# dmlc/difacto

Hardware: AMD Instinct MI355X
Metric: examples/sec (FM SGD worker step, Criteo-shape, V_dim=64) (higher is better)
Workload: dtype f32

## Files before the change

difacto_amd/capi.py:

```python
import ctypes as C
import os

import numpy as np

_HERE = os.path.dirname(os.path.abspath(__file__))
LIB_PATH = os.environ.get("DIFACTO_HIP_LIB") or os.path.join(_HERE, "libdifacto_hip.so")

FEA_COUNT, WEIGHT, GRADIENT = 1, 2, 3
INIT_REFRAND, INIT_HASH = 0, 1
U64MAX = 2 ** 64 - 1

SYMBOLS = [
    "dfh_last_error", "dfh_updater_param_default", "dfh_ctx_create", "dfh_ctx_destroy", "dfh_ctx_sync",
    "dfh_ctx_stream", "dfh_ctx_device", "dfh_reverse_bytes", "dfh_encode_fea_grp_id", "dfh_table_create",
    "dfh_table_destroy", "dfh_table_size", "dfh_table_param", "dfh_table_bytes", "dfh_pull", "dfh_push",
    "dfh_table_export", "dfh_table_import", "dfh_fm_predict", "dfh_fm_calcgrad", "dfh_loss_evaluate",
    "dfh_auc_times_n", "dfh_batch_create", "dfh_batch_destroy", "dfh_batch_load_host", "dfh_batch_load_device",
    "dfh_localize", "dfh_batch_load_localized_host", "dfh_batch_get_localized", "dfh_batch_shape", "dfh_sgd_step",
    "dfh_batch_progress", "dfh_batch_get_pred", "dfh_row_stride", "dfh_shard_pull", "dfh_shard_push_count",
    "dfh_shard_push_grad", "dfh_batch_forward", "dfh_batch_backward", "dfh_batch_device_keys", "dfh_malloc",
    "dfh_free", "dfh_memcpy_h2d", "dfh_memcpy_d2h", "dfh_ctx_set_timing", "dfh_ctx_get_timing", "dfh_kernel_name",
    "dfh_table_warm_start", "dfh_ctx_set_pipeline", "dfh_batch_lookup", "dfh_localize_lookup", "dfh_rowbuf_create", "dfh_rowbuf_destroy", "dfh_rowbuf_load_host", "dfh_batch_gather_rows", "dfh_batch_set_option", "dfh_batch_key_ranges", "dfh_batch_attach_device",
    "dfh_batch_key_ranges_device", "dfh_shard_resolve", "dfh_shard_pull_resolved", "dfh_shard_push_count_resolved",
    "dfh_shard_push_grad_resolved", "dfh_table_check", "dfh_ctx_set_timing_mask", "dfh_table_save", "dfh_table_load", "dfh_shard_resolve_multi", "dfh_shard_push_count_multi",
    "dfh_shard_push_grad_multi", "dfh_shard_count_pull_multi", "dfh_shard_push_grad_listed", "dfh_shard_release", "dfh_ctx_set_option", "dfh_table_set_has_aux", "dfh_table_has_aux",
    "dfh_comm_unique_id", "dfh_comm_create_rccl", "dfh_comm_create_callback", "dfh_comm_destroy", "dfh_comm_rank", "dfh_comm_world",
    "dfh_comm_allreduce_sum", "dfh_shard_create", "dfh_shard_destroy", "dfh_shard_owned_range", "dfh_shard_step", "dfh_shard_prefetch_counts",
    "dfh_shard_pull_host", "dfh_shard_push_host", "dfh_comm_allgather", "dfh_shard_balanced_splits", "dfh_shard_set_exchange", "dfh_shard_set_timing", "dfh_shard_get_timing",
    "dfh_comm_stats", "dfh_comm_info", "dfh_comm_selfcheck", "dfh_comm_wire_probe", "dfh_table_capacity", "dfh_batch_prepare_rows", "dfh_rowbuf_load_host_slices",
    "dfh_rowbuf_set_labels", "dfh_batch_prepare_cached", "dfh_batch_get_rows",
    "dfh_batch_create_many", "dfh_shard_multi_words", "dfh_shard_reserve", "dfh_comm_create_loopback", "dfh_comm_loopback_feed", "dfh_comm_loopback_wire", "dfh_comm_loopback_wire_time",
    "dfh_vec_inner_multi", "dfh_vec_combine", "dfh_vec_line_step", "dfh_lbfgs_create", "dfh_lbfgs_destroy", "dfh_lbfgs_add_chunk",
    "dfh_lbfgs_init_model", "dfh_lbfgs_shape", "dfh_lbfgs_get_model", "dfh_lbfgs_set_weights", "dfh_lbfgs_calc_grad",
    "dfh_lbfgs_prepare_direction", "dfh_lbfgs_calc_direction", "dfh_lbfgs_line_search", "dfh_lbfgs_evaluate", "dfh_lbfgs_create_sharded",
    "dfh_lbfgs_owned_range", "dfh_lbfgs_set_model", "dfh_bcd_set_model",
    "dfh_bcd_create", "dfh_bcd_destroy", "dfh_bcd_add_chunk", "dfh_bcd_build", "dfh_bcd_shape", "dfh_bcd_block_info",
    "dfh_bcd_epoch", "dfh_bcd_step", "dfh_bcd_get_model", "dfh_bcd_get_pred", "dfh_batch_split_entries",
    "dfh_bcd_create_sharded",
    "dfh_textchunk_create", "dfh_textchunk_destroy", "dfh_textchunk_parse_criteo", "dfh_textchunk_rows", "dfh_textchunk_ids",
    "dfh_rowbuf_load_slices",
]
XCHG_COUNTS, XCHG_KEYS, XCHG_CNT, XCHG_ROWS, XCHG_GRADS, XCHG_OTHER = range(6)
SHARD_STAGES = ("counts", "L", "K", "R", "RW", "F", "G", "P")
K_COUNT = 8
K_LOCALIZE, K_LOOKUP, K_FORWARD, K_BACKWARD, K_PULL, K_PUSH, K_MISC, K_AUC = range(8)


class UpdaterParam(C.Structure):
    _fields_ = [("l1", C.c_float), ("l2", C.c_float), ("V_l2", C.c_float), ("lr", C.c_float),
                ("lr_beta", C.c_float), ("V_lr", C.c_float), ("V_lr_beta", C.c_float),
                ("V_init_scale", C.c_float), ("V_dim", C.c_int), ("V_threshold", C.c_int),
                ("seed", C.c_uint), ("init_mode", C.c_int)]
# ... 56 lines not shown
    L.dfh_table_capacity.argtypes = [vp, PP(u64), PP(u64)]
    L.dfh_table_bytes.restype = u64
    L.dfh_table_bytes.argtypes = [vp]
    L.dfh_pull.argtypes = [vp, vp, sz, vp, PP(sz), vp, PP(sz)]
    L.dfh_push.argtypes = [vp, vp, sz, i32, vp, sz, vp, sz]
    L.dfh_table_export.argtypes = [vp, u64, vp, vp, vp, vp, PP(u64)]
    L.dfh_table_import.argtypes = [vp, u64, vp, vp, vp, vp]
    L.dfh_fm_predict.argtypes = [vp, i32, sz, vp, vp, vp, vp, sz, vp, vp, sz, vp]
    L.dfh_fm_calcgrad.argtypes = [vp, i32, sz, vp, vp, vp, vp, vp, sz, vp, vp, sz, vp, vp]
    L.dfh_loss_evaluate.argtypes = [vp, vp, vp, sz, PP(f32)]
    L.dfh_auc_times_n.argtypes = [vp, vp, vp, sz, PP(f32)]
    L.dfh_batch_create.argtypes = [vp, sz, sz, PP(vp)]
    L.dfh_batch_destroy.argtypes = [vp]
    L.dfh_batch_create_many.argtypes = [vp, i32, sz, sz, PP(vp)]
    L.dfh_batch_split_entries.argtypes = [vp, vp]
    L.dfh_batch_load_host.argtypes = [vp, sz, vp, vp, vp, vp]
    L.dfh_batch_load_device.argtypes = [vp, sz, sz, vp, vp, vp, vp]
    L.dfh_batch_attach_device.argtypes = [vp, sz, sz, vp, vp, vp, vp]
    L.dfh_localize.argtypes = [vp, u64]
    L.dfh_batch_load_localized_host.argtypes = [vp, sz, vp, vp, vp, vp, vp, vp, sz]
    L.dfh_batch_get_localized.argtypes = [vp, PP(sz), vp, vp, vp]
    L.dfh_batch_shape.argtypes = [vp, PP(sz), PP(sz), PP(sz)]
    L.dfh_sgd_step.argtypes = [vp, vp, i32, i32]
    L.dfh_batch_progress.argtypes = [vp, PP(Progress), i32]
    L.dfh_batch_get_pred.argtypes = [vp, vp]
    L.dfh_row_stride.restype = sz
    L.dfh_row_stride.argtypes = [i32]
    L.dfh_shard_pull.argtypes = [vp, vp, sz, vp]
    L.dfh_shard_push_count.argtypes = [vp, vp, sz, vp]
    L.dfh_shard_push_grad.argtypes = [vp, vp, sz, vp]
# ... 554 lines not shown
        p = Progress()
        _ck(lib().dfh_batch_progress(self.h, C.byref(p), 1 if reset else 0))
        return p

    def pred(self):
        nrows, _, _ = self.shape(want_U=False)
        out = np.zeros(nrows, np.float32)
        _ck(lib().dfh_batch_get_pred(self.h, _p(out)))
        return out

    def split_entries(self):
        n = C.c_uint32(0)
        _ck(lib().dfh_batch_split_entries(self.h, C.byref(n)))
        return int(n.value)

    def forward(self, V_dim, d_rows):
        _ck(lib().dfh_batch_forward(self.h, V_dim, _dp(d_rows)))

    def backward(self, V_dim, d_rows, d_grads):
        _ck(lib().dfh_batch_backward(self.h, V_dim, _dp(d_rows), _dp(d_grads)))

    def key_ranges(self, nparts):
        out = np.zeros(nparts + 1, np.uint32)
        _ck(lib().dfh_batch_key_ranges(self.h, nparts, _p(out)))
        return out

    def device_keys(self):
        a, b, u = C.c_void_p(), C.c_void_p(), C.c_size_t(0)
        _ck(lib().dfh_batch_device_keys(self.h, C.byref(a), C.byref(b), C.byref(u)))
        return a.value, b.value, u.value
# ... 388 lines not shown
```

difacto_amd/csrc/dfh_api.hip:

```cpp
#include <algorithm>
#include <chrono>
#include <cstring>
#include <mutex>
#include <new>
#include <thread>

#include <hip/hip_ext.h>
#include <rocprim/rocprim.hpp>

#include "dfh_kernels.hip"
#include "dfh_localize.hip"
#include "dfh_update.hip"
#include "dfh_riders.hip"

using namespace dfh;

namespace dfh {
static thread_local std::string g_err;
void set_error(const std::string& msg) { g_err = msg; }
}

struct dfh_ctx {
  int device = 0;
  hipStream_t stream = nullptr;
  bool own_stream = false;
  std::vector<hipStream_t> preps;
  std::vector<hipStream_t> extra;
  hipStream_t parse = nullptr;
  std::mutex parse_mu;
  unsigned nprep = 0;
  unsigned next_prep = 0;
  bool pipeline = false;
  void* scratch = nullptr;
  size_t scratch_bytes = 0;
  int num_cu = 256;
  int fwd_depth = 5;
  int fwd_blocks = 0;
  int bwd_small_blocks = 2048;
  int upd_kernel = 1;
  int upd_hot_blocks = 512, upd_mid_blocks = 512, upd_few_blocks = 1024, upd_single_blocks = 4096;
  int upd_interleave = 0;
  int owner_per_key = 0;
  int upd_split = 1;
  int auc_in_update = 1;
  int shard_mixed_update = 1;
  int grow_initial_rows = 1 << 20;
  int event_flags = 1;
  int prep_priority = -1;
  int single_queue = 0;
  int rider_slot[4] = {2, 0, 1, 2};
  int rider_alone[4] = {0, 0, 0, 0};
  int rider_period[3] = {1, 1, 1};
// ... 104 lines not shown
  uint32_t* d_split_ticket = nullptr;
  float* d_split_part = nullptr;
  size_t split_cap = 0;
  int split_sel = 0, split_last = 0;
  bool split_listing = false;
  uint32_t seg_nb = 0;
  uint2* d_uw = nullptr;
  uint32_t *d_urow = nullptr, *d_need = nullptr, *d_rank = nullptr, *d_total = nullptr;
  float *d_pred = nullptr, *d_slope = nullptr, *d_xv = nullptr;
  size_t xv_floats = 0;
  static constexpr size_t kProgDoubles = 2 * PROG_SLOTS + 64;
  double* d_prog = nullptr;
  float nrows_seen = 0;
  hipEvent_t ev_ready = nullptr, ev_free = nullptr;
  bool ready_pending = false, free_pending = false;
  hipStream_t prep = nullptr;
  bool compute_auc = false;
  uint32_t *d_auc_keys = nullptr, *d_auc_skeys = nullptr, *d_auc_lab = nullptr, *d_auc_slab = nullptr;
  uint32_t* d_auc_part = nullptr;
  uint32_t auc_pending_n = 0;
  bool force_radix = false;
  bool force_sort_fallback = false;
  dfh_table* looked_up = nullptr;
  struct GatherSeg { struct dfh_rowbuf* rb; size_t at, n; };
  std::vector<GatherSeg> gsegs;
  GatherSrc gsrc{};
  bool gather_pending = false, gather_fusable = false, gather_any_value = false, loc_fuse_gather = false;
  const uint32_t *g_rows = nullptr, *g_off = nullptr;
  const float* g_lab = nullptr;
  LocView loc_v{};
  EmitOut loc_o{};
// ... 3 lines not shown
};

namespace dfh {
namespace chunks {
inline hipError_t reset_prog(dfh_batch* b, hipStream_t s);
}
}

namespace {
int flush_pending(dfh_batch* b);
void pend_remove(dfh_ctx* c, dfh_batch* b);
inline hipStream_t prep_of(const dfh_batch* b) {
  const dfh_ctx* c = b->ctx;
  return (c->pipeline && b->prep) ? b->prep : c->stream;
}
void phase_begin(dfh_batch* b) {
  dfh_ctx* c = b->ctx;
  if (b->pend_stage < RID_STAGES) (void)flush_pending(b);
  hipStream_t next = c->pipeline ? c->preps[c->next_prep++ % c->nprep] : nullptr;
  if (next && b->prep && next != b->prep && b->ready_pending) {
    (void)hipStreamWaitEvent(next, b->ev_ready, 0);
  }
  b->prep = next;
}
int prep_begin(dfh_batch* b) {
  dfh_ctx* c = b->ctx;
  if (c->pipeline && !b->prep) phase_begin(b);
  if (c->pipeline && b->free_pending) {
    DFH_HIP(hipStreamWaitEvent(prep_of(b), b->ev_free, 0));
    b->free_pending = false;
  }
  return DFH_OK;
}
int prep_end(dfh_batch* b) {
  dfh_ctx* c = b->ctx;
  if (c->pipeline && !b->defer_ready) {
    DFH_HIP(hipEventRecord(b->ev_ready, prep_of(b)));
    b->ready_pending = true;
  }
  return DFH_OK;
}
int main_begin(dfh_batch* b) {
  dfh_ctx* c = b->ctx;
  if (b->pend_stage < RID_STAGES) {
    int rc = flush_pending(b);
    if (rc) return rc;
  }
  if (b->ready_pending) {
    DFH_HIP(hipStreamWaitEvent(c->stream, b->ev_ready, 0));
    b->ready_pending = false;
  }
  return DFH_OK;
}
int main_end(dfh_batch* b) {
  dfh_ctx* c = b->ctx;
  if (b->split_listing) {
    b->split_listing = false;
    b->split_last = b->split_sel;
    b->split_sel ^= 1;
  }
  if (c->pipeline) {
    DFH_HIP(hipEventRecord(b->ev_free, c->stream));
    b->free_pending = true;
// ... 14 lines not shown
  return SplitOut{b->d_split_ent, split_counter(b), u_base, (uint32_t)b->split_cap};
}
}

namespace {

inline int grid_for_threads(size_t n, const dfh_ctx* c) {
  size_t b = (n + 255) / 256;
  size_t cap = (size_t)c->num_cu * 8;
  return (int)std::max<size_t>(1, std::min(b, cap));
}
inline int grid_for_waves(size_t nwaves, const dfh_ctx* c) {
  size_t b = (nwaves + 3) / 4;
  size_t cap = (size_t)c->num_cu * 8;
  return (int)std::max<size_t>(1, std::min(b, cap));
}

int ensure_scratch(dfh_ctx* c, size_t bytes) {
  if (bytes <= c->scratch_bytes) return DFH_OK;
  if (c->scratch) {
    DFH_HIP(hipStreamSynchronize(c->stream));
    DFH_HIP(hipFree(c->scratch));
    c->scratch = nullptr;
    c->scratch_bytes = 0;
  }
  size_t want = std::max(bytes, (size_t)1 << 20);
  want = (want + 255) & ~(size_t)255;
  DFH_HIP(hipMalloc(&c->scratch, want));
  c->scratch_bytes = want;
  return DFH_OK;
// ... 486 lines not shown

inline int count_mode(const dfh_ctx* c, int is_train, int push_cnt) { return push_cnt ? ((is_train && c->upd_kernel) ? 2 : 1) : 0; }

struct StepExtras {
  uint32_t* need = nullptr;
  bool pre = false;
  bool riders = false;
  bool spans = false;
};

int step_lookup(dfh_table* t, dfh_batch* b, int is_train, int push_cnt, uint32_t lo, const uint32_t* d_n, size_t n, const StepExtras& x,
                const float* rrows = nullptr, size_t U = 0, hipEvent_t rows_in = nullptr) {
  dfh_ctx* c = t->ctx;
  hipStream_t s = c->stream;
  const float* cnt = b->has_cnt ? b->d_feacnt + lo : (const float*)nullptr;
  const int mode = count_mode(c, is_train, push_cnt), gl = grid_for_threads(n, c);
  const uint32_t n_static = d_n ? 0u : (uint32_t)n;
  static const bool gap_trace = getenv("DFH_GAP_TRACE") != nullptr;
  const bool ride = x.spans && gap_trace && ((c->timing >> DFH_K_LOOKUP) & 1u);
  TimeScope ts(c, (x.spans && !ride) ? DFH_K_LOOKUP : DFH_K_COUNT);
  const SplitOut so = split_out(c, b, is_train, lo);
  RiderSet rs;
  rs.n = 0;
  if (x.riders) collect_riders(c, 0, true, ((uint32_t)gl + 7u) / 8u, &rs);
  if (rrows) {
    DFH_HIP(hipStreamWaitEvent(s, rows_in, 0));
    const UwRemote m{rrows, dfh_row_stride(t->v.k), b->d_U, lo, lo + (uint32_t)n, b->d_uw, b->d_col_ptr, split_out(c, b, is_train, 0u), t->v.err};
    hipLaunchKernelGGL(k_lookup_uw_remote, dim3(grid_for_threads(U, c)), dim3(256), 0, s, t->v, b->d_feaids + lo, n_static, b->d_urow + lo,
                       cnt, b->d_col_ptr + lo, mode, b->d_uw + lo, auc_pending(b), m, so);
  } else if (rs.n) {
    hipLaunchKernelGGL(k_lookup_riders, dim3((((unsigned)gl + 7u) / 8u + rs.ngroups) * 8u), dim3(256), rider_smem(rs), s, t->v,
// ... 156 lines not shown
  delete c;
  return DFH_OK;
}

int dfh_ctx_sync(dfh_ctx* c) {
  DFH_ARG(c, "ctx is NULL");
  return sync_all(c);
}

int dfh_ctx_set_pipeline(dfh_ctx* c, int enable) {
  DFH_ARG(c, "ctx is NULL");
  DFH_ARG(enable >= 0 && enable <= 4, "dfh_ctx_set_pipeline: 0 (off) .. 4 preparation streams");
  if (c->single_queue && enable) {
    return DFH_OK;
  }
  int rc = sync_all(c);
  if (rc) return rc;
  while ((int)c->preps.size() < enable) {
    int lo = 0, hi = 0;
    DFH_HIP(hipDeviceGetStreamPriorityRange(&lo, &hi));
    const int prio = c->prep_priority < 0 ? lo : (c->prep_priority > 0 ? hi : 0);
    hipStream_t p = nullptr;
    DFH_HIP(hipStreamCreateWithPriority(&p, hipStreamNonBlocking, prio));
    c->preps.push_back(p);
  }
  c->nprep = (unsigned)enable;
  c->next_prep = 0;
  c->pipeline = enable != 0;
  return DFH_OK;
}
int dfh_ctx_set_option(dfh_ctx* c, const char* name, int value) {
  DFH_ARG(c && name, "dfh_ctx_set_option: NULL argument");
  const std::string n(name);
  if (n == "fwd_depth") {
    DFH_ARG(value == 4 || value == 5 || value == 8 || value == 10, "fwd_depth must be 4, 5, 8 or 10");
    c->fwd_depth = value;
  } else if (n == "fwd_blocks") {
    DFH_ARG(value >= 0 && value <= PROG_SLOTS, "fwd_blocks must be in [0, 16384] (0: one wave per example)");
    c->fwd_blocks = value;
  } else if (n == "bwd_small_blocks") {
    DFH_ARG(value >= 1 && value <= 65536, "bwd_small_blocks must be in [1, 65536]");
    c->bwd_small_blocks = value;
  } else if (n == "upd_kernel") {
    DFH_ARG(value == 0 || value == 1, "upd_kernel must be 0 (k_backward_all) or 1 (k_update_fused)");
    c->upd_kernel = value;
  } else if (n == "upd_hot_blocks" || n == "upd_mid_blocks" || n == "upd_few_blocks" || n == "upd_single_blocks") {
    DFH_ARG(value >= 1 && value <= 65536, "upd_*_blocks must be in [1, 65536]");
    (n == "upd_hot_blocks" ? c->upd_hot_blocks : n == "upd_mid_blocks" ? c->upd_mid_blocks : n == "upd_few_blocks" ? c->upd_few_blocks
                                                                                                        : c->upd_single_blocks) = value;
  } else if (n == "grow_initial_rows") {
    DFH_ARG(value >= 16 && value <= (1 << 28), "grow_initial_rows must be in [16, 2^28]");
    c->grow_initial_rows = value;
  } else if (n == "auc_in_update") {
    DFH_ARG(value == 0 || value == 1, "auc_in_update must be 0 (k_auc_pairs as its own launch) or 1 (a role of k_update_fused)");
// ... 8 lines not shown
    DFH_ARG(value == 0 || value == 1, "upd_split must be 0 (one block per hot key, whatever its length) or 1 (a block per part of 1 024 occurrences)");
    c->upd_split = value;
  } else if (n == "upd_interleave") {
    DFH_ARG(value >= 0 && value <= 64, "upd_interleave must be in [0, 64]");
    c->upd_interleave = value;
  } else if (n == "event_flags") {
    DFH_ARG(value == 0 || value == 1, "event_flags must be 0 (default events) or 1 (no system-scope fence); set before batches are created");
    c->event_flags = value;
  } else if (n == "single_queue") {
    DFH_ARG(value == 0 || value == 1, "single_queue must be 0 (preparation streams) or 1 (the Localizer's stages ride in the step's launches)");
    if (value != c->single_queue) {
      for (dfh_batch* p : std::vector<dfh_batch*>(c->pend)) {
        int rcf = flush_pending(p);
        if (rcf) return rcf;
      }
      int rcs = sync_all(c);
      if (rcs) return rcs;
      if (value) {
        c->nprep = 0;
        c->next_prep = 0;
        c->pipeline = false;
      }
      c->single_queue = value;
    }
  } else if (n == "rider_slot_count" || n == "rider_slot_scatter" || n == "rider_slot_sort" || n == "rider_slot_emit") {
    DFH_ARG(value >= 0 && value <= 6 && (value & 3) <= 2, "rider_slot_*: 0 lookup, 1 forward, 2 update (+ 4: alone, before that launch)");
    const int st = n == "rider_slot_count" ? 0 : n == "rider_slot_scatter" ? 1 : n == "rider_slot_sort" ? 2 : 3;
    c->rider_slot[st] = value & 3;
    c->rider_alone[st] = (value >> 2) & 1;
  } else if (n == "rider_start_lookup" || n == "rider_start_forward" || n == "rider_start_update") {
    DFH_ARG(value >= 0 && value <= 100, "rider_start_*: per cent of the carrier's own blocks dispatched before the first rider group");
// ... 1124 lines not shown
  }
  if (--sa->refs == 0) {
    hipFree(sa->base);
    delete sa;
  }
  return rc;
}

int dfh_batch_destroy(dfh_batch* b) {
  if (b && b->n_prof)
    fprintf(stderr, "dfh_batch_prepare_rows x %llu: begin %.4f s, wait staged %.4f, write description %.4f, gather %.4f, localize %.4f, lookup + ready %.4f\n",
            (unsigned long long)b->n_prof, b->t_prof[0], b->t_prof[1], b->t_prof[2], b->t_prof[3], b->t_prof[4], b->t_prof[5]);
  if (!b) return DFH_OK;
  hipSetDevice(b->ctx->device);
  pend_remove(b->ctx, b);
  sync_all(b->ctx);
  if (b->ev_ready) hipEventDestroy(b->ev_ready);
  if (b->ev_free) hipEventDestroy(b->ev_free);
  if (b->ev_staged) hipEventDestroy(b->ev_staged);
  if (b->h_stage) hipHostFree(b->h_stage);
  if (b->d_xv) hipFree(b->d_xv);
  if (b->arena) hipFree(b->arena);
  if (b->shared_arena) {
    SharedArena* sa = static_cast<SharedArena*>(b->shared_arena);
    if (--sa->refs == 0) {
      hipFree(sa->base);
      delete sa;
    }
  }
  delete b;
// ... 292 lines not shown
  } else {
    hipLaunchKernelGGL(k_rdx_keys, dim3(g), dim3(256), 0, s, b->d_raw, N, max_index, b->d_keys, b->d_pos);
    size_t tb = b->temp_bytes;
    DFH_HIP(rocprim::radix_sort_pairs(b->d_temp, tb, b->d_keys, b->d_skeys, b->d_pos, b->d_spos, (size_t)N, 0, 64, s));
    hipLaunchKernelGGL(k_rdx_heads, dim3(g), dim3(256), 0, s, b->d_skeys, N, b->d_head);
    tb = b->temp_bytes;
    DFH_HIP(rocprim::inclusive_scan(b->d_temp, tb, b->d_head, b->d_uid, (size_t)N, rocprim::plus<uint32_t>(), s));
    hipLaunchKernelGGL(k_rdx_emit, dim3(g), dim3(256), 0, s, b->d_skeys, b->d_spos, b->d_head, b->d_uid, N, (uint32_t)b->nrows,
                       b->d_offset, b->has_value ? b->d_value : (const float*)nullptr, b->d_feaids, b->d_col_ptr, b->d_index,
                       b->d_s_row, b->d_s_val, b->d_U);
    hipLaunchKernelGGL(k_seg_lists_reset, dim3(1), dim3(64), 0, s, b->d_mid, b->d_hot, b->d_few, b->d_U + 2);
    hipLaunchKernelGGL(k_seg_lists, dim3((unsigned)std::max<size_t>(1, std::min<size_t>((N + 1023) / 1024, 256))), dim3(1024), 0, s,
                       b->d_col_ptr, b->d_U, b->d_mid, b->d_hot, b->d_few, b->d_mid_ent, b->d_hot_ent, b->d_few_ent);
    b->seg_nb = 1;
    if (probe)
      hipLaunchKernelGGL(k_lookup, dim3(grid_for_threads(b->nnz, c)), dim3(256), 0, s, probe->v, b->d_feaids, b->d_U, 0u, b->d_urow,
                         (const float*)nullptr, b->d_col_ptr, 0, (uint32_t*)nullptr, 0, (uint2*)nullptr, AucFin{nullptr, 0u, nullptr});
  }
  delete tsp;
  DFH_HIP(hipGetLastError());
  b->localized = true;
  b->has_cnt = false;
  if (probe) b->looked_up = probe;
  return prep_end(b);
}
}


int dfh_localize(dfh_batch* b, uint64_t max_index) {
  DFH_ARG(b && b->nrows > 0, "dfh_localize: no batch loaded");
  DFH_ARG(max_index != 0, "max_index must be nonzero");
// ... 35 lines not shown
    set_error("dfh_batch_lookup: batch is not localized");
    return DFH_ERR_STATE;
  }
  dfh_ctx* c = b->ctx;
  if (b->nnz == 0) return DFH_OK;
  if (b->nnz <= kSmallBatchPairs) return DFH_OK;
  if (c->single_queue) return DFH_OK;
  DFH_HIP(hipSetDevice(c->device));
  int rc = table_reserve(t, b->nnz);
  if (rc) return rc;
  rc = prep_begin(b);
  if (rc) return rc;
  {
    hipStream_t ps = prep_of(b);
    TimeScope ts(c, DFH_K_LOOKUP, ps);
    hipLaunchKernelGGL(k_lookup, dim3(grid_for_threads(b->nnz, c)), dim3(256), 0, ps, t->v, b->d_feaids, b->d_U, 0u,
                       b->d_urow, (const float*)nullptr, b->d_col_ptr, 0, (uint32_t*)nullptr, 0, (uint2*)nullptr, AucFin{nullptr, 0u, nullptr});
  }
  DFH_HIP(hipGetLastError());
  b->looked_up = t;
  return prep_end(b);
}

int dfh_batch_load_localized_host(dfh_batch* b, size_t nrows, const size_t* offset, const uint32_t* index, const float* value,
                                  const float* label, const uint64_t* feaids, const float* feacnt, size_t U) {
  DFH_ARG(b && offset && label && feaids, "dfh_batch_load_localized_host: NULL argument");
  DFH_ARG(nrows >= 1 && nrows <= b->max_rows, "nrows out of range");
  std::vector<uint32_t> off32;
  int rc = to_u32_offsets(offset, nrows, &off32);
  if (rc) return rc;
  const size_t base = offset[0], nnz = off32[nrows];
// ... 37 lines not shown
  DFH_HIP(hipMemcpyAsync(b->d_label, label, nrows * 4, hipMemcpyHostToDevice, s));
  if (U) DFH_HIP(hipMemcpyAsync(b->d_feaids, feaids, U * 8, hipMemcpyHostToDevice, s));
  if (U && feacnt) DFH_HIP(hipMemcpyAsync(b->d_feacnt, feacnt, U * 4, hipMemcpyHostToDevice, s));
  DFH_HIP(hipMemcpyAsync(b->d_col_ptr, col_ptr.data(), (U + 1) * 4, hipMemcpyHostToDevice, s));
  DFH_HIP(hipMemcpyAsync(b->d_U, &U32, 4, hipMemcpyHostToDevice, s));
  hipLaunchKernelGGL(k_seg_lists_reset, dim3(1), dim3(64), 0, s, b->d_mid, b->d_hot, b->d_few, b->d_U + 2);
  if (U) {
    hipLaunchKernelGGL(k_seg_lists, dim3((unsigned)std::min<size_t>((U + 1023) / 1024, 256)), dim3(1024), 0, s, b->d_col_ptr,
                       b->d_U, b->d_mid, b->d_hot, b->d_few, b->d_mid_ent, b->d_hot_ent, b->d_few_ent);
  }
  b->seg_nb = 1;
  DFH_HIP(hipGetLastError());
  DFH_HIP(hipStreamSynchronize(s));
  b->nrows = nrows;
  b->nnz = nnz;
  b->has_value = value != nullptr;
  b->has_cnt = feacnt != nullptr;
  b->localized = true;
  return prep_end(b);
}

int dfh_batch_shape(dfh_batch* b, size_t* nrows, size_t* nnz, size_t* U) {
  DFH_ARG(b, "NULL batch");
  if (nrows) *nrows = b->nrows;
  if (nnz) *nnz = b->nnz;
  if (U) {
    DFH_ARG(b->localized, "batch is not localized");
    uint32_t u = 0;
    int rc = flush_pending(b);
    if (rc) return rc;
    rc = sync_all(b->ctx);
    if (rc) return rc;
    DFH_HIP(hipMemcpyAsync(&u, b->d_U, 4, hipMemcpyDeviceToHost, b->ctx->stream));
    DFH_HIP(hipStreamSynchronize(b->ctx->stream));
    *U = u;
  }
  return DFH_OK;
}

int dfh_batch_get_localized(dfh_batch* b, size_t* U, uint64_t* feaids, float* feacnt, uint32_t* index) {
  DFH_ARG(b && b->localized, "batch is not localized");
  size_t u = 0;
  int rc = dfh_batch_shape(b, nullptr, nullptr, &u);
  if (rc) return rc;
  if (U) *U = u;
  hipStream_t s = b->ctx->stream;
  if (feaids && u) DFH_HIP(hipMemcpyAsync(feaids, b->d_feaids, u * 8, hipMemcpyDeviceToHost, s));
  if (feacnt && u) {
    if (!b->has_cnt) {
      hipLaunchKernelGGL(k_loc_counts, dim3(grid_for_threads(u, b->ctx)), dim3(256), 0, s, b->d_col_ptr, b->d_U, b->d_feacnt);
// ... 109 lines not shown
  if (is_train && refrand) {
    rc = refrand_flush(t, b->d_feaids, b->d_U, Nb, b->d_urow, b->d_need, b->d_rank, b->d_total);
    if (rc) return rc;
  }
  return main_end(b);
}

int dfh_batch_split_entries(dfh_batch* b, uint32_t* n) {
  DFH_ARG(b && n, "dfh_batch_split_entries: NULL argument");
  dfh_ctx* c = b->ctx;
  DFH_HIP(hipSetDevice(c->device));
  if (b->pend_stage < RID_STAGES) {
    int rc = flush_pending(b);
    if (rc) return rc;
  }
  if (b->ready_pending) DFH_HIP(hipStreamWaitEvent(c->stream, b->ev_ready, 0));
  DFH_HIP(hipMemcpyAsync(n, b->d_U + 2 + b->split_last, sizeof(uint32_t), hipMemcpyDeviceToHost, c->stream));
  DFH_HIP(hipStreamSynchronize(c->stream));
  return DFH_OK;
}

int dfh_batch_forward(dfh_batch* b, int V_dim, const float* d_rows) {
  DFH_ARG(b && b->localized && d_rows, "dfh_batch_forward: bad argument");
  const int kp = (V_dim + 3) / 4 * 4;
  int rc = ensure_xv(b, kp);
  if (rc) return rc;
  b->nrows_seen += (float)b->nrows;
  rc = main_begin(b);
  if (rc) return rc;
  rc = launch_forward(b, packed_src(d_rows, V_dim), V_dim, kp);
  if (rc) return rc;
  return main_end(b);
// ... 100 lines not shown
```

difacto_amd/csrc/dfh_feed.hip:

```cpp
struct dfh_rowbuf {
  dfh_ctx* ctx = nullptr;
  size_t max_rows = 0, max_nnz = 0, nrows = 0, nnz = 0;
  uint32_t* d_off = nullptr;
  uint64_t* d_idx = nullptr;
  float* d_val = nullptr;
  float* d_lab = nullptr;
  bool has_value = false, has_labels = false;
  hipStream_t up = nullptr;
  hipEvent_t ev_loaded = nullptr;
  struct Used { hipStream_t stream; hipEvent_t ev; bool pending; };
  std::mutex mu;
  std::vector<Used> used;
  std::vector<hipStream_t> seen_loaded;
  double t_prof[3] = {0, 0, 0};
  uint64_t n_prof = 0, bytes_prof = 0;
  std::vector<uint32_t> off32;
};

namespace {
int localize_impl(dfh_batch* b, uint64_t max_index, dfh_table* probe);

struct PrepLaps {
  double* acc;
  bool on;
// ... 303 lines not shown
  gs.dst_off = b->d_offset;
  gs.dst_lab = b->d_label;
  batch_loaded(b, nrows, in.nnz, in.any_value);
  return DFH_OK;
}

int queue_described(dfh_table* t, dfh_batch* b, const DescribedIn& in, uint64_t max_index, PrepLaps& laps) {
  dfh_ctx* c = b->ctx;
  int rc = describe(b, in);
  if (rc) return rc;
  laps.lap(3);
  b->defer_ready = true;
  rc = localize_impl(b, max_index, nullptr);
  laps.lap(4);
  if (!rc && in.nnz > kSmallBatchPairs && !c->single_queue) {
    hipLaunchKernelGGL(k_lookup, dim3(grid_for_threads(b->nnz, c)), dim3(256), 0, prep_of(b), t->v, b->d_feaids, b->d_U, 0u, b->d_urow,
                       (const float*)nullptr, b->d_col_ptr, 0, (uint32_t*)nullptr, 0, (uint2*)nullptr, AucFin{nullptr, 0u, nullptr});
    if (hipGetLastError() != hipSuccess) rc = DFH_ERR_HIP;
    b->looked_up = t;
  }
  b->defer_ready = false;
  if (rc) return rc;
  rc = prep_end(b);
  laps.lap(5);
  if (laps.on) ++b->n_prof;
  return rc;
}
}

extern "C" {

// ... 224 lines not shown
```

difacto_amd/csrc/dfh_internal.h:

```cpp
#ifndef DFH_INTERNAL_H_
#define DFH_INTERNAL_H_
#include <hip/hip_runtime.h>
#include <stdint.h>
#include <string>
#include <vector>

#include "difacto_hip.h"

namespace dfh {

constexpr int kWave = 64;
constexpr uint64_t kEmptyKey = ~0ULL;
constexpr uint32_t kNoRow = ~0u;

struct __attribute__((aligned(16))) HEntry {
  uint64_t key;
  uint32_t row;
  uint32_t pad;
};

struct __attribute__((aligned(32))) RowHdr {
  float w;
  uint32_t has_V;
  float sqrt_g;
// ... 28 lines not shown
  const uint2* few;
  const SegEnt* few_ent;
  const SegEnt* split_ent;
  const uint32_t* split_n;
};
#ifndef DFH_HOT_SPLIT
#define DFH_HOT_SPLIT 1024
#endif
#ifndef DFH_HOT_SPLIT_MIN
#define DFH_HOT_SPLIT_MIN 4096
#endif
constexpr uint32_t HOT_SPLIT = DFH_HOT_SPLIT;
constexpr uint32_t HOT_SPLIT_MIN = DFH_HOT_SPLIT_MIN;
#ifndef DFH_HOT_SPLIT_BUILD
#define DFH_HOT_SPLIT_BUILD 3
#endif

constexpr uint32_t kRemoteRow = 0x80000000u;
constexpr uint32_t kSingleRow = 0x40000000u;
constexpr uint32_t kCountLater = 0x20000000u;
constexpr uint32_t kHasV = 0x10000000u;
constexpr uint32_t kRowMask = 0x0FFFFFFFu;

struct RowSrc {
  const float* wbase;
  size_t wstride;
  const float* vbase;
  size_t vstride;
  const uint32_t* urow;
  int flag_is_float;
// ... 59 lines not shown
```

difacto_amd/csrc/dfh_kernels.hip:

```cpp
#include "dfh_internal.h"

namespace dfh {

__device__ __forceinline__ int lane_id() { return threadIdx.x & 63; }

__device__ __forceinline__ float wave_sum(float v) {
#pragma unroll
  for (int o = 32; o > 0; o >>= 1) v += __shfl_xor(v, o, 64);
  return v;
}

template <int L>
__device__ __forceinline__ float cross_group_sum(float v) {
#pragma unroll
  for (int o = L; o < 64; o <<= 1) v += __shfl_xor(v, o, 64);
  return v;
}
template <int L>
__device__ __forceinline__ float in_group_sum(float v) {
#pragma unroll
  for (int o = L >> 1; o > 0; o >>= 1) v += __shfl_xor(v, o, 64);
  return v;
}

// ... 379 lines not shown
  uint32_t cap;
};
__device__ __forceinline__ uint32_t* split_other(uint32_t* n) { return reinterpret_cast<uint32_t*>(reinterpret_cast<uintptr_t>(n) ^ 4u); }
__device__ __forceinline__ void lookup_split(const SplitOut& so, uint32_t* err, uint32_t u, uint32_t beg, uint32_t end) {
  if (!(DFH_HOT_SPLIT_BUILD & 1) || !so.ent || end - beg <= HOT_SPLIT_MIN) return;
  const uint32_t nparts = (end - beg + HOT_SPLIT - 1u) / HOT_SPLIT;
  const uint32_t base = atomicAdd(so.n, nparts);
  if (base + nparts > so.cap) {
    atomicOr(err, 16u);
    return;
  }
  for (uint32_t p = 0; p < nparts; ++p)
    so.ent[base + p] = make_uint4(u + so.u_base, beg + p * HOT_SPLIT, min(beg + (p + 1u) * HOT_SPLIT, end), (p << 16) | nparts);
}

template <bool SPLIT = true>
__device__ __forceinline__ void lookup_body(const TableView& t, const uint64_t* __restrict__ keys, const uint32_t* __restrict__ d_n,
                         uint32_t n_static, uint32_t* __restrict__ urow, const float* __restrict__ cnt,
                         const uint32_t* __restrict__ col_ptr, int push_cnt, uint32_t* __restrict__ need_init,
                         int rows_known, uint2* __restrict__ uw, AucFin fin, const uint32_t bid, const uint32_t nblk,
                         const SplitOut so = SplitOut{nullptr, nullptr, 0u, 0u}) {
  if (fin.n && bid == 0) auc_finalize_block(fin);
  if (SPLIT && so.n && bid == 0 && threadIdx.x == 0) *split_other(so.n) = 0u;
  uint32_t n = d_n ? *d_n : n_static;
  __shared__ uint32_t ins_sh[8];
  for (uint32_t u0 = bid * blockDim.x; u0 < n; u0 += nblk * blockDim.x) {
    const uint32_t u = u0 + threadIdx.x;
    const bool active = u < n;
    uint64_t key = active ? keys[u] : 0ull;
    uint32_t r;
    if (rows_known) r = active ? (urow[u] & kRowMask) : 0u;
    else if (blockDim.x == 256) r = find_or_insert_block(t, key, active, ins_sh);
    else r = active ? find_or_insert(t, key) : 0u;
    if (!active) continue;
    if (urow && !rows_known) urow[u] = r;
    if (SPLIT && col_ptr) lookup_split(so, t.err, u, col_ptr[u], col_ptr[u + 1]);
    float w = 0.f;
    bool hasv = false;
    if (push_cnt) {
// ... 29 lines not shown
      uw[u] = make_uint2(r | (single ? kSingleRow : 0u) | (hasv ? kHasV : 0u), __float_as_uint(w));
    }
  }
}

__global__ void k_lookup(TableView t, const uint64_t* __restrict__ keys, const uint32_t* __restrict__ d_n,
                         uint32_t n_static, uint32_t* __restrict__ urow, const float* __restrict__ cnt,
                         const uint32_t* __restrict__ col_ptr, int push_cnt, uint32_t* __restrict__ need_init,
                         int rows_known, uint2* __restrict__ uw, AucFin fin) {
  lookup_body<false>(t, keys, d_n, n_static, urow, cnt, col_ptr, push_cnt, need_init, rows_known, uw, fin, blockIdx.x, gridDim.x);
}
__global__ void k_lookup_step(TableView t, const uint64_t* __restrict__ keys, const uint32_t* __restrict__ d_n,
                              uint32_t n_static, uint32_t* __restrict__ urow, const float* __restrict__ cnt,
                              const uint32_t* __restrict__ col_ptr, int push_cnt, uint32_t* __restrict__ need_init,
                              int rows_known, uint2* __restrict__ uw, AucFin fin, SplitOut so) {
  lookup_body<true>(t, keys, d_n, n_static, urow, cnt, col_ptr, push_cnt, need_init, rows_known, uw, fin, blockIdx.x, gridDim.x, so);
}

struct UwRemote {
  const float* rows;
  size_t stride;
  const uint32_t* d_U;
  uint32_t lo, hi;
  uint2* uw;
  const uint32_t* col_ptr;
  SplitOut so;
  uint32_t* err;
};
__device__ __forceinline__ void uw_remote_body(const UwRemote& m) {
  const uint32_t U = *m.d_U;
  if (m.so.n && blockIdx.x == 0 && threadIdx.x == 0) *split_other(m.so.n) = 0u;
// ... 1711 lines not shown
```

difacto_amd/csrc/dfh_shard.hip:

```cpp
#ifndef DFH_SHARD_HIP_
#define DFH_SHARD_HIP_
#include <dlfcn.h>
#include <link.h>

#include <chrono>
#include <deque>
#include <optional>
#include <thread>

namespace dfh {

struct RcclId { char internal[128]; };
struct RcclApi {
  void* lib = nullptr;
  int (*GetUniqueId)(RcclId*) = nullptr;
  int (*CommInitRank)(void**, int, RcclId, int) = nullptr;
  int (*CommDestroy)(void*) = nullptr;
  const char* (*GetErrorString)(int) = nullptr;
  int (*Send)(const void*, size_t, int, int, void*, hipStream_t) = nullptr;
  int (*Recv)(void*, size_t, int, int, void*, hipStream_t) = nullptr;
  int (*GroupStart)() = nullptr;
  int (*GroupEnd)() = nullptr;
  int (*GetVersion)(int*) = nullptr;
  std::string path;
// ... 1066 lines not shown
int shard_step_overlap(dfh_shard* s, dfh_batch* b, int is_train, int push_cnt, int* any_active) {
  dfh_comm* c = s->c;
  dfh_ctx* ctx = s->t->ctx;
  DFH_HIP(hipSetDevice(ctx->device));
  hipStream_t st = ctx->stream, cs = s->cs;
  int rc;
  if (s->timing) ++s->stage_steps;
  static const bool trace = getenv("DFH_SHARD_TRACE") != nullptr;
  Flight& cur = s->fl[s->cur];
  if (trace)
    fprintf(stderr, "[shard %d] step %llu: b=%p cur{slot %d described %d pulled %d b=%p} armed %d next_b=%p\n", c->rank,
            (unsigned long long)s->steps, (void*)b, s->cur, (int)cur.described, (int)cur.pulled, (void*)cur.b, (int)s->next_armed,
            (void*)s->next_b);
  if (!(cur.described && cur.b == b)) {
    DFH_ARG(!cur.described || !cur.pulled, "dfh_shard_step: the batch differs from the one announced to dfh_shard_prefetch_counts");
    if (b && b->ready_pending) DFH_HIP(hipStreamWaitEvent(cs, b->ev_ready, 0));
    {
      StageScope ts(s, DFH_SHARD_STAGE_COUNTS, cs);
      rc = queue_counts(s, b, cs);
      if (rc) return rc;
    }
    DFH_HIP(hipStreamSynchronize(cs));
    flight_sizes(s, cur, b, s->cur);
  }
  if (any_active) *any_active = cur.active != 0 ? 1 : 0;
  ++s->steps;
  if (b) b->nrows_seen += (float)b->nrows;
  const bool look = s->next_armed;
  dfh_batch* nb = look ? s->next_b : nullptr;
  s->next_armed = false;
  Flight& nxt = s->fl[s->cur ^ 1];
  nxt = Flight();
  if (cur.active == 0) {
    cur = Flight();
    return b ? main_end(b) : DFH_OK;
  }
  auto keys_out = [&](Flight& f) {
    const int q = f.slot;
    hipEvent_t ready = f.b && f.b->ready_pending ? f.b->ev_ready : nullptr;
    hipEvent_t freed = s->p_pending[q] ? s->ev_p[q] : nullptr;
    s->p_pending[q] = false;
    return flight_K(s, f, push_cnt, cs, ready, freed, s->ev_k[q]);
  };
  auto rows_back = [&](Flight& f) {
    const int q = f.slot;
    int r = flight_R(s, f, push_cnt, s->ev_k[q], s->ev_r[q]);
    if (!r) r = flight_RW(s, f, cs, s->ev_r[q], s->ev_rw[q]);
    f.pulled = r == DFH_OK;
    return r;
  };
  rc = flight_bufs(s, cur);
  if (rc) return rc;
  if (b) {
    rc = main_begin(b);
    if (rc) return rc;
  }
  const int q = cur.slot;
  const bool uw_folded = cur.any_own && cur.pulled && cur.any_remote && b != nullptr;
  if ((rc = flight_L(s, cur, is_train, push_cnt, uw_folded ? s->ev_rw[q] : nullptr))) return rc;
  if (!cur.pulled) {
    if ((rc = keys_out(cur)) || (rc = rows_back(cur))) return rc;
  }
  if (look) {
    if (nb && nb->ready_pending) DFH_HIP(hipStreamWaitEvent(cs, nb->ev_ready, 0));
    StageScope ts(s, DFH_SHARD_STAGE_COUNTS, cs);
    rc = queue_counts(s, nb, cs);
    if (rc) return rc;
    DFH_HIP(hipEventRecord(s->cnt_ev, cs));
  }
  if ((rc = flight_F(s, cur, is_train, push_cnt, uw_folded, uw_folded ? nullptr : s->ev_rw[q], s->ev_f))) return rc;
  bool ahead = false;
  if (look) {
    DFH_HIP(hipEventSynchronize(s->cnt_ev));
    flight_sizes(s, nxt, nb, s->cur ^ 1);
    ahead = nxt.active != 0;
    if (trace)
      fprintf(stderr, "[shard %d]   next: active %zu U %zu nrecv %zu own [%u, %u) -> ahead %d\n", c->rank, nxt.active, nxt.U, nxt.nrecv,
              nxt.own_lo, nxt.own_hi, (int)ahead);
// ... 319 lines not shown
```

include/difacto_hip.h:

```cpp
#ifndef DIFACTO_HIP_H_
#define DIFACTO_HIP_H_
#include <stddef.h>
#include <stdint.h>

#ifdef __cplusplus
extern "C" {
#endif

enum {
  DFH_OK = 0,
  DFH_ERR_ARG = 1,
  DFH_ERR_HIP = 2,
  DFH_ERR_CAPACITY = 3,
  DFH_ERR_STATE = 4
};

enum { DFH_FEA_COUNT = 1, DFH_WEIGHT = 2, DFH_GRADIENT = 3 };

enum {
  DFH_INIT_REFRAND = 0,
  DFH_INIT_HASH = 1
};

typedef struct {
// ... 115 lines not shown
int dfh_rowbuf_set_labels(dfh_rowbuf* rb, size_t nrows, const float* label);
int dfh_batch_prepare_cached(dfh_table* t, dfh_batch* b, size_t nrows, int nseg, dfh_rowbuf* const* bufs, const uint32_t* const* rows,
                             const size_t* seg_rows, uint64_t max_index);

int dfh_batch_load_localized_host(dfh_batch* b, size_t nrows, const size_t* offset, const uint32_t* index,
                                  const float* value, const float* label, const uint64_t* feaids,
                                  const float* feacnt, size_t U);
int dfh_batch_get_localized(dfh_batch* b, size_t* U, uint64_t* feaids, float* feacnt, uint32_t* index);
int dfh_batch_shape(dfh_batch* b, size_t* nrows, size_t* nnz, size_t* U);
int dfh_batch_get_rows(dfh_batch* b, uint32_t* offset, float* label);

int dfh_sgd_step(dfh_table* t, dfh_batch* b, int is_train, int push_cnt);
int dfh_batch_progress(dfh_batch* b, dfh_progress* out, int reset);
int dfh_batch_get_pred(dfh_batch* b, float* pred);
int dfh_batch_split_entries(dfh_batch* b, uint32_t* n);

size_t dfh_row_stride(int V_dim);
int dfh_shard_pull(dfh_table* t, const uint64_t* d_keys, size_t n, float* d_rows);
int dfh_shard_push_count(dfh_table* t, const uint64_t* d_keys, size_t n, const float* d_cnt);
int dfh_shard_push_grad(dfh_table* t, const uint64_t* d_keys, size_t n, const float* d_grads);
int dfh_batch_forward(dfh_batch* b, int V_dim, const float* d_rows);
int dfh_batch_backward(dfh_batch* b, int V_dim, const float* d_rows, float* d_grads);
int dfh_batch_device_keys(dfh_batch* b, const uint64_t** d_feaids, const float** d_feacnt, size_t* U);
int dfh_batch_key_ranges(dfh_batch* b, int nparts, uint32_t* bounds);
int dfh_batch_key_ranges_device(dfh_batch* b, int nparts, const uint64_t* d_splits, int64_t* d_bounds);

int dfh_shard_resolve(dfh_table* t, const uint64_t* d_keys, size_t n, uint32_t* d_rowid);
int dfh_shard_pull_resolved(dfh_table* t, const uint32_t* d_rowid, size_t n, float* d_rows);
int dfh_shard_push_count_resolved(dfh_table* t, const uint32_t* d_rowid, const uint64_t* d_keys, size_t n, const float* d_cnt);
int dfh_shard_push_grad_resolved(dfh_table* t, const uint32_t* d_rowid, const uint64_t* d_keys, size_t n, const float* d_grads);
// ... 104 lines not shown
```

Baseline: 88.05 million.

## Defer ready-event records, size lookup grids by unique count, pair rows in lookup

Pipelined prep streams no longer record the batch-ready event at prep end right away. The event is recorded lazily when another batch reuses that stream or a consumer needs it, which cuts event-record calls. Lookup kernel grids are now sized from a unique-key hint capped at a configurable number of blocks per CU, instead of from nnz. The known-rows lookup path handles two unique keys per thread so their header loads overlap. A debug accessor for row words is also added. Together these add bookkeeping complexity and ordering risk around when events get recorded.

```diff
diff --git a/difacto_amd/capi.py b/difacto_amd/capi.py
--- a/difacto_amd/capi.py
+++ b/difacto_amd/capi.py
@@ -36,6 +36,7 @@
     "dfh_lbfgs_owned_range", "dfh_lbfgs_set_model", "dfh_bcd_set_model",
     "dfh_bcd_create", "dfh_bcd_destroy", "dfh_bcd_add_chunk", "dfh_bcd_build", "dfh_bcd_shape", "dfh_bcd_block_info",
     "dfh_bcd_epoch", "dfh_bcd_step", "dfh_bcd_get_model", "dfh_bcd_get_pred", "dfh_batch_split_entries",
+    "dfh_batch_get_row_words",
     "dfh_bcd_create_sharded",
     "dfh_textchunk_create", "dfh_textchunk_destroy", "dfh_textchunk_parse_criteo", "dfh_textchunk_rows", "dfh_textchunk_ids",
     "dfh_rowbuf_load_slices",
@@ -122,6 +123,8 @@
     L.dfh_batch_destroy.argtypes = [vp]
     L.dfh_batch_create_many.argtypes = [vp, i32, sz, sz, PP(vp)]
     L.dfh_batch_split_entries.argtypes = [vp, vp]
+    if hasattr(L, "dfh_batch_get_row_words"):
+        L.dfh_batch_get_row_words.argtypes = [vp, sz, vp, vp]
     L.dfh_batch_load_host.argtypes = [vp, sz, vp, vp, vp, vp]
     L.dfh_batch_load_device.argtypes = [vp, sz, sz, vp, vp, vp, vp]
     L.dfh_batch_attach_device.argtypes = [vp, sz, sz, vp, vp, vp, vp]
@@ -706,6 +709,12 @@
         _ck(lib().dfh_batch_split_entries(self.h, C.byref(n)))
         return int(n.value)
 
+    def row_words(self, U):
+        urow = np.zeros(max(U, 1), np.uint32)
+        uw = np.zeros(max(U, 1), np.uint64)
+        _ck(lib().dfh_batch_get_row_words(self.h, U, _p(urow), _p(uw)))
+        return urow[:U], uw[:U]
+
     def forward(self, V_dim, d_rows):
         _ck(lib().dfh_batch_forward(self.h, V_dim, _dp(d_rows)))
 
diff --git a/difacto_amd/csrc/dfh_api.hip b/difacto_amd/csrc/dfh_api.hip
--- a/difacto_amd/csrc/dfh_api.hip
+++ b/difacto_amd/csrc/dfh_api.hip
@@ -31,11 +31,13 @@
   unsigned nprep = 0;
   unsigned next_prep = 0;
   bool pipeline = false;
+  std::vector<dfh_batch*> owed;
   void* scratch = nullptr;
   size_t scratch_bytes = 0;
   int num_cu = 256;
   int fwd_depth = 5;
   int fwd_blocks = 0;
+  int lookup_waves = 3;
   int bwd_small_blocks = 2048;
   int upd_kernel = 1;
   int upd_hot_blocks = 512, upd_mid_blocks = 512, upd_few_blocks = 1024, upd_single_blocks = 4096;
@@ -170,7 +172,9 @@
   float nrows_seen = 0;
   hipEvent_t ev_ready = nullptr, ev_free = nullptr;
   bool ready_pending = false, free_pending = false;
+  hipStream_t owed_on = nullptr;
   hipStream_t prep = nullptr;
+  size_t u_hint = 0;
   bool compute_auc = false;
   uint32_t *d_auc_keys = nullptr, *d_auc_skeys = nullptr, *d_auc_lab = nullptr, *d_auc_slab = nullptr;
   uint32_t* d_auc_part = nullptr;
@@ -204,11 +208,40 @@
   const dfh_ctx* c = b->ctx;
   return (c->pipeline && b->prep) ? b->prep : c->stream;
 }
+inline dfh_batch** owed_slot(dfh_ctx* c, hipStream_t s) {
+  for (size_t i = 0; i < c->preps.size() && i < c->owed.size(); ++i)
+    if (c->preps[i] == s) return &c->owed[i];
+  return nullptr;
+}
+int ready_settle(dfh_batch* b) {
+  if (!b->owed_on) return DFH_OK;
+  hipStream_t s = b->owed_on;
+  b->owed_on = nullptr;
+  dfh_batch** slot = owed_slot(b->ctx, s);
+  if (slot && *slot == b) *slot = nullptr;
+  DFH_HIP(hipEventRecord(b->ev_ready, s));
+  return DFH_OK;
+}
+int ready_settle_others(dfh_batch* b, hipStream_t s) {
+  dfh_batch** slot = owed_slot(b->ctx, s);
+  if (slot && *slot && *slot != b) return ready_settle(*slot);
+  return DFH_OK;
+}
+int ready_settle_all(dfh_ctx* c) {
+  for (dfh_batch* o : std::vector<dfh_batch*>(c->owed))
+    if (o) {
+      int rc = ready_settle(o);
+      if (rc) return rc;
+    }
+  return DFH_OK;
+}
 void phase_begin(dfh_batch* b) {
   dfh_ctx* c = b->ctx;
   if (b->pend_stage < RID_STAGES) (void)flush_pending(b);
   hipStream_t next = c->pipeline ? c->preps[c->next_prep++ % c->nprep] : nullptr;
+  if (next) (void)ready_settle_others(b, next);
   if (next && b->prep && next != b->prep && b->ready_pending) {
+    (void)ready_settle(b);
     (void)hipStreamWaitEvent(next, b->ev_ready, 0);
   }
   b->prep = next;
@@ -216,6 +249,10 @@
 int prep_begin(dfh_batch* b) {
   dfh_ctx* c = b->ctx;
   if (c->pipeline && !b->prep) phase_begin(b);
+  if (c->pipeline) {
+    int rc = ready_settle_others(b, prep_of(b));
+    if (rc) return rc;
+  }
   if (c->pipeline && b->free_pending) {
     DFH_HIP(hipStreamWaitEvent(prep_of(b), b->ev_free, 0));
     b->free_pending = false;
@@ -225,7 +262,22 @@
 int prep_end(dfh_batch* b) {
   dfh_ctx* c = b->ctx;
   if (c->pipeline && !b->defer_ready) {
-    DFH_HIP(hipEventRecord(b->ev_ready, prep_of(b)));
+    hipStream_t s = prep_of(b);
+    if (b->owed_on && b->owed_on != s) {
+      int rc = ready_settle(b);
+      if (rc) return rc;
+    }
+    dfh_batch** slot = owed_slot(c, s);
+    if (slot) {
+      if (*slot && *slot != b) {
+        int rc = ready_settle(*slot);
+        if (rc) return rc;
+      }
+      *slot = b;
+      b->owed_on = s;
+    } else {
+      DFH_HIP(hipEventRecord(b->ev_ready, s));
+    }
     b->ready_pending = true;
   }
   return DFH_OK;
@@ -237,6 +289,8 @@
     if (rc) return rc;
   }
   if (b->ready_pending) {
+    int rc = ready_settle(b);
+    if (rc) return rc;
     DFH_HIP(hipStreamWaitEvent(c->stream, b->ev_ready, 0));
     b->ready_pending = false;
   }
@@ -281,6 +335,15 @@
   size_t b = (nwaves + 3) / 4;
   size_t cap = (size_t)c->num_cu * 8;
   return (int)std::max<size_t>(1, std::min(b, cap));
+}
+inline int lookup_grid(const dfh_ctx* c, const dfh_batch* b, size_t bound, bool exact) {
+  size_t hint = bound;
+  if (!exact) {
+    if (b->u_hint) hint = std::min(hint, b->u_hint);
+    hint = std::max(hint, b->nnz / 4);
+  }
+  const size_t blocks = (hint + 255) / 256, cap = (size_t)c->num_cu * (size_t)c->lookup_waves;
+  return (int)std::max<size_t>(1, std::min(blocks, cap));
 }
 
 int ensure_scratch(dfh_ctx* c, size_t bytes) {
@@ -797,7 +860,7 @@
   dfh_ctx* c = t->ctx;
   hipStream_t s = c->stream;
   const float* cnt = b->has_cnt ? b->d_feacnt + lo : (const float*)nullptr;
-  const int mode = count_mode(c, is_train, push_cnt), gl = grid_for_threads(n, c);
+  const int mode = count_mode(c, is_train, push_cnt), gl = lookup_grid(c, b, n, d_n == nullptr);
   const uint32_t n_static = d_n ? 0u : (uint32_t)n;
   static const bool gap_trace = getenv("DFH_GAP_TRACE") != nullptr;
   const bool ride = x.spans && gap_trace && ((c->timing >> DFH_K_LOOKUP) & 1u);
@@ -984,7 +1047,9 @@
   if (c->single_queue && enable) {
     return DFH_OK;
   }
-  int rc = sync_all(c);
+  int rc = ready_settle_all(c);
+  if (rc) return rc;
+  rc = sync_all(c);
   if (rc) return rc;
   while ((int)c->preps.size() < enable) {
     int lo = 0, hi = 0;
@@ -994,6 +1059,7 @@
     DFH_HIP(hipStreamCreateWithPriority(&p, hipStreamNonBlocking, prio));
     c->preps.push_back(p);
   }
+  c->owed.resize(c->preps.size(), nullptr);
   c->nprep = (unsigned)enable;
   c->next_prep = 0;
   c->pipeline = enable != 0;
@@ -1008,6 +1074,9 @@
   } else if (n == "fwd_blocks") {
     DFH_ARG(value >= 0 && value <= PROG_SLOTS, "fwd_blocks must be in [0, 16384] (0: one wave per example)");
     c->fwd_blocks = value;
+  } else if (n == "lookup_waves") {
+    DFH_ARG(value >= 1 && value <= 8, "lookup_waves must be in [1, 8] (blocks per CU the lookup passes' grids are capped at)");
+    c->lookup_waves = value;
   } else if (n == "bwd_small_blocks") {
     DFH_ARG(value >= 1 && value <= 65536, "bwd_small_blocks must be in [1, 65536]");
     c->bwd_small_blocks = value;
@@ -1046,7 +1115,8 @@
         int rcf = flush_pending(p);
         if (rcf) return rcf;
       }
-      int rcs = sync_all(c);
+      int rcs = ready_settle_all(c);
+      if (!rcs) rcs = sync_all(c);
       if (rcs) return rcs;
       if (value) {
         c->nprep = 0;
@@ -2201,6 +2271,7 @@
   if (!b) return DFH_OK;
   hipSetDevice(b->ctx->device);
   pend_remove(b->ctx, b);
+  (void)ready_settle(b);
   sync_all(b->ctx);
   if (b->ev_ready) hipEventDestroy(b->ev_ready);
   if (b->ev_free) hipEventDestroy(b->ev_free);
@@ -2523,7 +2594,7 @@
                        b->d_col_ptr, b->d_U, b->d_mid, b->d_hot, b->d_few, b->d_mid_ent, b->d_hot_ent, b->d_few_ent);
     b->seg_nb = 1;
     if (probe)
-      hipLaunchKernelGGL(k_lookup, dim3(grid_for_threads(b->nnz, c)), dim3(256), 0, s, probe->v, b->d_feaids, b->d_U, 0u, b->d_urow,
+      hipLaunchKernelGGL(k_lookup, dim3(lookup_grid(c, b, b->nnz, false)), dim3(256), 0, s, probe->v, b->d_feaids, b->d_U, 0u, b->d_urow,
                          (const float*)nullptr, b->d_col_ptr, 0, (uint32_t*)nullptr, 0, (uint2*)nullptr, AucFin{nullptr, 0u, nullptr});
   }
   delete tsp;
@@ -2589,7 +2660,7 @@
   {
     hipStream_t ps = prep_of(b);
     TimeScope ts(c, DFH_K_LOOKUP, ps);
-    hipLaunchKernelGGL(k_lookup, dim3(grid_for_threads(b->nnz, c)), dim3(256), 0, ps, t->v, b->d_feaids, b->d_U, 0u,
+    hipLaunchKernelGGL(k_lookup, dim3(lookup_grid(c, b, b->nnz, false)), dim3(256), 0, ps, t->v, b->d_feaids, b->d_U, 0u,
                        b->d_urow, (const float*)nullptr, b->d_col_ptr, 0, (uint32_t*)nullptr, 0, (uint2*)nullptr, AucFin{nullptr, 0u, nullptr});
   }
   DFH_HIP(hipGetLastError());
@@ -2657,6 +2728,7 @@
   DFH_HIP(hipStreamSynchronize(s));
   b->nrows = nrows;
   b->nnz = nnz;
+  b->u_hint = U;
   b->has_value = value != nullptr;
   b->has_cnt = feacnt != nullptr;
   b->localized = true;
@@ -2677,6 +2749,7 @@
     DFH_HIP(hipMemcpyAsync(&u, b->d_U, 4, hipMemcpyDeviceToHost, b->ctx->stream));
     DFH_HIP(hipStreamSynchronize(b->ctx->stream));
     *U = u;
+    b->u_hint = u;
   }
   return DFH_OK;
 }
@@ -2816,8 +2889,24 @@
     int rc = flush_pending(b);
     if (rc) return rc;
   }
-  if (b->ready_pending) DFH_HIP(hipStreamWaitEvent(c->stream, b->ev_ready, 0));
+  if (b->ready_pending) {
+    int rc = ready_settle(b);
+    if (rc) return rc;
+    DFH_HIP(hipStreamWaitEvent(c->stream, b->ev_ready, 0));
+  }
   DFH_HIP(hipMemcpyAsync(n, b->d_U + 2 + b->split_last, sizeof(uint32_t), hipMemcpyDeviceToHost, c->stream));
+  DFH_HIP(hipStreamSynchronize(c->stream));
+  return DFH_OK;
+}
+
+int dfh_batch_get_row_words(dfh_batch* b, size_t n, uint32_t* urow, uint64_t* uw) {
+  DFH_ARG(b && b->localized && n <= b->max_nnz, "dfh_batch_get_row_words: bad argument");
+  dfh_ctx* c = b->ctx;
+  DFH_HIP(hipSetDevice(c->device));
+  int rc = sync_all(c);
+  if (rc) return rc;
+  if (urow && n) DFH_HIP(hipMemcpyAsync(urow, b->d_urow, n * sizeof(uint32_t), hipMemcpyDeviceToHost, c->stream));
+  if (uw && n) DFH_HIP(hipMemcpyAsync(uw, b->d_uw, n * sizeof(uint2), hipMemcpyDeviceToHost, c->stream));
   DFH_HIP(hipStreamSynchronize(c->stream));
   return DFH_OK;
 }
diff --git a/difacto_amd/csrc/dfh_feed.hip b/difacto_amd/csrc/dfh_feed.hip
--- a/difacto_amd/csrc/dfh_feed.hip
+++ b/difacto_amd/csrc/dfh_feed.hip
@@ -341,7 +341,7 @@
   rc = localize_impl(b, max_index, nullptr);
   laps.lap(4);
   if (!rc && in.nnz > kSmallBatchPairs && !c->single_queue) {
-    hipLaunchKernelGGL(k_lookup, dim3(grid_for_threads(b->nnz, c)), dim3(256), 0, prep_of(b), t->v, b->d_feaids, b->d_U, 0u, b->d_urow,
+    hipLaunchKernelGGL(k_lookup, dim3(lookup_grid(c, b, b->nnz, false)), dim3(256), 0, prep_of(b), t->v, b->d_feaids, b->d_U, 0u, b->d_urow,
                        (const float*)nullptr, b->d_col_ptr, 0, (uint32_t*)nullptr, 0, (uint2*)nullptr, AucFin{nullptr, 0u, nullptr});
     if (hipGetLastError() != hipSuccess) rc = DFH_ERR_HIP;
     b->looked_up = t;
diff --git a/difacto_amd/csrc/dfh_internal.h b/difacto_amd/csrc/dfh_internal.h
--- a/difacto_amd/csrc/dfh_internal.h
+++ b/difacto_amd/csrc/dfh_internal.h
@@ -66,6 +66,9 @@
 constexpr uint32_t HOT_SPLIT_MIN = DFH_HOT_SPLIT_MIN;
 #ifndef DFH_HOT_SPLIT_BUILD
 #define DFH_HOT_SPLIT_BUILD 3
+#endif
+#ifndef DFH_LOOKUP_PAIR
+#define DFH_LOOKUP_PAIR 1
 #endif
 
 constexpr uint32_t kRemoteRow = 0x80000000u;
diff --git a/difacto_amd/csrc/dfh_kernels.hip b/difacto_amd/csrc/dfh_kernels.hip
--- a/difacto_amd/csrc/dfh_kernels.hip
+++ b/difacto_amd/csrc/dfh_kernels.hip
@@ -417,7 +417,39 @@
     so.ent[base + p] = make_uint4(u + so.u_base, beg + p * HOT_SPLIT, min(beg + (p + 1u) * HOT_SPLIT, end), (p << 16) | nparts);
 }
 
-template <bool SPLIT = true>
+template <bool SPLIT>
+__device__ __forceinline__ void lookup_known(const TableView& t, const uint64_t* __restrict__ keys, const float* __restrict__ cnt,
+                                             int push_cnt, uint32_t* __restrict__ need_init, uint2* __restrict__ uw, const SplitOut& so,
+                                             uint32_t u, uint32_t r, uint32_t beg, uint32_t end, uint2 wh) {
+  if (SPLIT) lookup_split(so, t.err, u, beg, end);
+  const float w = __uint_as_float(wh.x);
+  const uint32_t single = end - beg == 1u ? kSingleRow : 0u;
+  bool hasv = wh.y != 0u;
+  if (push_cnt) {
+    if (hasv) {
+      if (need_init) need_init[u] = 0u;
+      uw[u] = make_uint2(r | kCountLater | kHasV | single, wh.x);
+      return;
+    }
+    const float c = cnt ? cnt[u] : (float)(end - beg);
+    RowHdr& h = t.hdr[r];
+    const float fc = h.fea_cnt + c;
+    h.fea_cnt = fc;
+    const bool init = t.k > 0 && w != 0 && fc > (float)t.p.V_threshold;
+    if (t.p.init_mode == DFH_INIT_HASH) {
+      if (init) {
+        init_v_hash_row(t, r, keys[u]);
+        h.has_V = 1;
+      }
+    } else if (need_init) {
+      need_init[u] = init ? 1u : 0u;
+    }
+    hasv = init;
+  }
+  uw[u] = make_uint2(r | single | (hasv ? kHasV : 0u), wh.x);
+}
+
+template <bool SPLIT = true, bool PAIR = false>
 __device__ __forceinline__ void lookup_body(const TableView& t, const uint64_t* __restrict__ keys, const uint32_t* __restrict__ d_n,
                          uint32_t n_static, uint32_t* __restrict__ urow, const float* __restrict__ cnt,
                          const uint32_t* __restrict__ col_ptr, int push_cnt, uint32_t* __restrict__ need_init,
@@ -426,6 +458,20 @@
   if (fin.n && bid == 0) auc_finalize_block(fin);
   if (SPLIT && so.n && bid == 0 && threadIdx.x == 0) *split_other(so.n) = 0u;
   uint32_t n = d_n ? *d_n : n_static;
+  if (PAIR && rows_known && uw && col_ptr && push_cnt != 1) {
+    const uint32_t stride = nblk * blockDim.x;
+    for (uint32_t u = bid * blockDim.x + threadIdx.x; u < n; u += 2u * stride) {
+      const uint32_t v = u + stride;
+      const bool two = v < n;
+      const uint32_t ra = urow[u] & kRowMask, a0 = col_ptr[u], a1 = col_ptr[u + 1];
+      const uint32_t rb = two ? (urow[v] & kRowMask) : 0u, b0 = two ? col_ptr[v] : 0u, b1 = two ? col_ptr[v + 1] : 0u;
+      const uint2 wa = *reinterpret_cast<const uint2*>(&t.hdr[ra]);
+      const uint2 wb = two ? *reinterpret_cast<const uint2*>(&t.hdr[rb]) : make_uint2(0u, 0u);
+      lookup_known<SPLIT>(t, keys, cnt, push_cnt, need_init, uw, so, u, ra, a0, a1, wa);
+      if (two) lookup_known<SPLIT>(t, keys, cnt, push_cnt, need_init, uw, so, v, rb, b0, b1, wb);
+    }
+    return;
+  }
   __shared__ uint32_t ins_sh[8];
   for (uint32_t u0 = bid * blockDim.x; u0 < n; u0 += nblk * blockDim.x) {
     const uint32_t u = u0 + threadIdx.x;
@@ -485,7 +531,8 @@
                               uint32_t n_static, uint32_t* __restrict__ urow, const float* __restrict__ cnt,
                               const uint32_t* __restrict__ col_ptr, int push_cnt, uint32_t* __restrict__ need_init,
                               int rows_known, uint2* __restrict__ uw, AucFin fin, SplitOut so) {
-  lookup_body<true>(t, keys, d_n, n_static, urow, cnt, col_ptr, push_cnt, need_init, rows_known, uw, fin, blockIdx.x, gridDim.x, so);
+  lookup_body<true, DFH_LOOKUP_PAIR != 0>(t, keys, d_n, n_static, urow, cnt, col_ptr, push_cnt, need_init, rows_known, uw, fin, blockIdx.x,
+                                          gridDim.x, so);
 }
 
 struct UwRemote {
diff --git a/difacto_amd/csrc/dfh_shard.hip b/difacto_amd/csrc/dfh_shard.hip
--- a/difacto_amd/csrc/dfh_shard.hip
+++ b/difacto_amd/csrc/dfh_shard.hip
@@ -1104,6 +1104,7 @@
             (void*)s->next_b);
   if (!(cur.described && cur.b == b)) {
     DFH_ARG(!cur.described || !cur.pulled, "dfh_shard_step: the batch differs from the one announced to dfh_shard_prefetch_counts");
+    if (b && b->ready_pending && (rc = ready_settle(b))) return rc;
     if (b && b->ready_pending) DFH_HIP(hipStreamWaitEvent(cs, b->ev_ready, 0));
     {
       StageScope ts(s, DFH_SHARD_STAGE_COUNTS, cs);
@@ -1127,6 +1128,7 @@
   }
   auto keys_out = [&](Flight& f) {
     const int q = f.slot;
+    if (f.b && f.b->ready_pending && ready_settle(f.b)) return (int)DFH_ERR_HIP;
     hipEvent_t ready = f.b && f.b->ready_pending ? f.b->ev_ready : nullptr;
     hipEvent_t freed = s->p_pending[q] ? s->ev_p[q] : nullptr;
     s->p_pending[q] = false;
@@ -1152,6 +1154,7 @@
     if ((rc = keys_out(cur)) || (rc = rows_back(cur))) return rc;
   }
   if (look) {
+    if (nb && nb->ready_pending && (rc = ready_settle(nb))) return rc;
     if (nb && nb->ready_pending) DFH_HIP(hipStreamWaitEvent(cs, nb->ev_ready, 0));
     StageScope ts(s, DFH_SHARD_STAGE_COUNTS, cs);
     rc = queue_counts(s, nb, cs);
diff --git a/include/difacto_hip.h b/include/difacto_hip.h
--- a/include/difacto_hip.h
+++ b/include/difacto_hip.h
@@ -153,6 +153,7 @@
 int dfh_batch_progress(dfh_batch* b, dfh_progress* out, int reset);
 int dfh_batch_get_pred(dfh_batch* b, float* pred);
 int dfh_batch_split_entries(dfh_batch* b, uint32_t* n);
+int dfh_batch_get_row_words(dfh_batch* b, size_t n, uint32_t* urow, uint64_t* uw);
 
 size_t dfh_row_stride(int V_dim);
 int dfh_shard_pull(dfh_table* t, const uint64_t* d_keys, size_t n, float* d_rows);
```

Measured after the change: 88.34 million, median of 2. About the same (+0.3%).
